# a1q123456/image_stitching

Hardware: AMD Instinct MI355X
Metric: 4K frames stitched/sec (higher is better)
Workload: dtype u8

## Files before the change

image_stitching_amd/csrc/orb.hip:

```cpp
#include "common.h"
#include "dev_math.h"
#include <algorithm>
#include <cmath>
#include <mutex>
#include <unordered_map>

#define ORB_MAX_LEVELS 16
#define ORB_BORDER 32

namespace {

struct LevelDesc {
    int w, h;
    int pp;
    int sp;
    size_t pad_off;
    size_t map_off;
    float scale;
    int nfeat;
    int n2;
    int tiles_x, tiles_y, tile_off;
    int cap1, cand_off;
    int cap2, fin_off;
    int tab_off;
};

struct Levels {
    int n;
    int fast_t, patch, half_patch, edge;
    LevelDesc d[ORB_MAX_LEVELS];
};

struct Work {
    uint8_t *pad, *blur, *score, *nms;
    int* hist;
    int* thr;
    int* tile_cnt;
    uint32_t* surv_xy;
    uint8_t* surv_sc;
    int* cnt1;
    int* cnt2;
    int* flags;
    uint32_t* cand_xy;
    float* cand_resp;
    uint32_t* fin_xy;
    float* fin_resp;
    int* tab;
    int* umax;
    int8_t* pattern;
};

constexpr int ORB_BATCH = 16;
struct OrbIO {
    const uint8_t* src[ORB_BATCH];
    size_t sstride[ORB_BATCH];
    int aligned[ORB_BATCH];
    MisKeyPoint* kps[ORB_BATCH];
    uint32_t* lxy[ORB_BATCH];
    int* n_dev[ORB_BATCH];
    uint8_t* desc[ORB_BATCH];
};
#define WS_OFF(p, f, ws) p = (decltype(p))((const char*)(p) + (size_t)(f) * (ws))

constexpr int GRAY_ROWS = 4;
__global__ __launch_bounds__(256) void gray_kernel(OrbIO io, int w, int h, uint8_t* dst, int pp, size_t ws) {
    const int x = (blockIdx.x * 256 + threadIdx.x) * 4, y0 = blockIdx.y * GRAY_ROWS, f = blockIdx.z;
    if (x >= w) return;
    const uint8_t* bgr = io.src[f];
    const size_t stride = io.sstride[f];
    const int aligned = io.aligned[f];
    WS_OFF(dst, f, ws);
    const int nrows = min(GRAY_ROWS, h - y0);
    if (aligned && x + 4 <= w) {
        unsigned w0[GRAY_ROWS], w1[GRAY_ROWS], w2[GRAY_ROWS];
#pragma unroll
        for (int r = 0; r < GRAY_ROWS; r++) {
            const unsigned* sp = reinterpret_cast<const unsigned*>(bgr + (size_t)min(y0 + r, h - 1) * stride + 3 * (size_t)x);
            w0[r] = sp[0]; w1[r] = sp[1]; w2[r] = sp[2];
        }
#pragma unroll
        for (int r = 0; r < GRAY_ROWS; r++) {
            if (r >= nrows) break;
            const unsigned g0 = ((w0[r] & 255) * 3735 + ((w0[r] >> 8) & 255) * 19235 + ((w0[r] >> 16) & 255) * 9798 + (1 << 14)) >> 15;
            const unsigned g1 = ((w0[r] >> 24) * 3735 + (w1[r] & 255) * 19235 + ((w1[r] >> 8) & 255) * 9798 + (1 << 14)) >> 15;
            const unsigned g2 = (((w1[r] >> 16) & 255) * 3735 + (w1[r] >> 24) * 19235 + (w2[r] & 255) * 9798 + (1 << 14)) >> 15;
            const unsigned g3 = (((w2[r] >> 8) & 255) * 3735 + ((w2[r] >> 16) & 255) * 19235 + (w2[r] >> 24) * 9798 + (1 << 14)) >> 15;
            *reinterpret_cast<unsigned*>(dst + (size_t)(y0 + r + ORB_BORDER) * pp + ORB_BORDER + x) = g0 | (g1 << 8) | (g2 << 16) | (g3 << 24);
        }
    } else {
        for (int r = 0; r < nrows; r++) {
            const uint8_t* s = bgr + (size_t)(y0 + r) * stride + 3 * (size_t)x;
            uint8_t* o = dst + (size_t)(y0 + r + ORB_BORDER) * pp + ORB_BORDER + x;
            for (int k = 0; k < 4 && x + k < w; k++) o[k] = (uint8_t)((s[3 * k] * 3735 + s[3 * k + 1] * 19235 + s[3 * k + 2] * 9798 + (1 << 14)) >> 15);
        }
    }
}

__device__ __forceinline__ unsigned byte_at(unsigned w0, unsigned w1, unsigned w2, int o) {
    const unsigned long long lo = (unsigned long long)w0 | ((unsigned long long)w1 << 32);
    return (o < 8 ? (unsigned)(lo >> (8 * o)) : (w2 >> (8 * (o - 8)))) & 255u;
}
#ifndef MIS_RS_ROWS
#define MIS_RS_ROWS 4
#endif
constexpr int RS_ROWS = MIS_RS_ROWS;
__global__ __launch_bounds__(256) void resize_kernel(const uint8_t* __restrict__ src, int sw, int sh, int spp, uint8_t* __restrict__ dst, int dw, int dh, int dpp,
                                                     const int* __restrict__ tab, size_t ws) {
    const int x = (blockIdx.x * 64 + (threadIdx.x & 63)) * 4;
    const int ybase = __builtin_amdgcn_readfirstlane((blockIdx.y * 4 + (threadIdx.x >> 6)) * RS_ROWS);
    if (x >= dw || ybase >= dh) return;
    WS_OFF(src, blockIdx.z, ws); WS_OFF(dst, blockIdx.z, ws);
    const int dw4 = (dw + 3) & ~3;
    const int *xo = tab, *xm = tab + dw4, *yo = tab + 2 * dw4, *ym = tab + 2 * dw4 + dh;
    const int4 o4 = *reinterpret_cast<const int4*>(xo + x), m4 = *reinterpret_cast<const int4*>(xm + x);
    const int xs[4] = {o4.x, o4.y, o4.z, o4.w}, ms[4] = {m4.x, m4.y, m4.z, m4.w};
    const int nvalid = min(4, dw - x), nrows = min(RS_ROWS, dh - ybase);
    const int base = xs[0] & ~3, last = xs[nvalid - 1] + 1 - base;
    const uint8_t* r0[RS_ROWS];
    const uint8_t* r1[RS_ROWS];
    int my1[RS_ROWS];
#pragma unroll
    for (int r = 0; r < RS_ROWS; r++) {
        const int y = min(ybase + r, dh - 1);
        const int y0 = yo[y], y1 = y0 + 1 < sh ? y0 + 1 : y0;
        my1[r] = ym[y];
        r0[r] = src + (size_t)(y0 + ORB_BORDER) * spp + ORB_BORDER;
        r1[r] = src + (size_t)(y1 + ORB_BORDER) * spp + ORB_BORDER;
    }
    uint8_t* out = dst + (size_t)(ybase + ORB_BORDER) * dpp + ORB_BORDER + x;
    unsigned res[RS_ROWS];
    if (last <= 11) {
        unsigned a[RS_ROWS][3], b[RS_ROWS][3];
#pragma unroll
        for (int r = 0; r < RS_ROWS; r++) {
            const unsigned* p0 = reinterpret_cast<const unsigned*>(r0[r] + base);
            const unsigned* p1 = reinterpret_cast<const unsigned*>(r1[r] + base);
            a[r][0] = p0[0]; a[r][1] = p0[1]; a[r][2] = p0[2]; b[r][0] = p1[0]; b[r][1] = p1[1]; b[r][2] = p1[2];
        }
#pragma unroll
        for (int r = 0; r < RS_ROWS; r++) res[r] = 0;
#pragma unroll
        for (int k = 0; k < 4; k++) {
            const int o = xs[k] - base, mx1 = ms[k], mx0 = 256 - mx1;
            const bool ok = k < nvalid;
            const int oo = ok ? o : 0;
            const bool p1 = oo >= 4, p2 = oo >= 8;
#pragma unroll
            for (int r = 0; r < RS_ROWS; r++) {
                const unsigned alo = p2 ? a[r][2] : (p1 ? a[r][1] : a[r][0]), ahi = p2 ? 0u : (p1 ? a[r][2] : a[r][1]);
                const unsigned blo = p2 ? b[r][2] : (p1 ? b[r][1] : b[r][0]), bhi = p2 ? 0u : (p1 ? b[r][2] : b[r][1]);
                const unsigned ta = __builtin_amdgcn_alignbyte(ahi, alo, (unsigned)oo & 3u), tb = __builtin_amdgcn_alignbyte(bhi, blo, (unsigned)oo & 3u);
                const unsigned h0 = (ta & 255u) * mx0 + ((ta >> 8) & 255u) * mx1;
                const unsigned h1 = (tb & 255u) * mx0 + ((tb >> 8) & 255u) * mx1;
                res[r] |= ok ? ((h0 * (256 - my1[r]) + h1 * my1[r] + (1u << 15)) >> 16) << (8 * k) : 0u;
            }
        }
    } else {
#pragma unroll
        for (int r = 0; r < RS_ROWS; r++) {
            res[r] = 0;
#pragma unroll
            for (int k = 0; k < 4; k++) {
                if (k >= nvalid) break;
                const int x0 = xs[k], x1 = x0 + 1 < sw ? x0 + 1 : x0, mx1 = ms[k], mx0 = 256 - mx1;
                const unsigned h0 = (unsigned)r0[r][x0] * mx0 + (unsigned)r0[r][x1] * mx1;
                const unsigned h1 = (unsigned)r1[r][x0] * mx0 + (unsigned)r1[r][x1] * mx1;
                res[r] |= ((h0 * (256 - my1[r]) + h1 * my1[r] + (1u << 15)) >> 16) << (8 * k);
            }
        }
    }
#pragma unroll
    for (int r = 0; r < RS_ROWS; r++) {
        if (r >= nrows) break;
        uint8_t* o = out + (size_t)r * dpp;
        if (nvalid == 4) *reinterpret_cast<unsigned*>(o) = res[r];
        else
            for (int k = 0; k < nvalid; k++) o[k] = (uint8_t)(res[r] >> (8 * k));
    }
}

template <bool SIDES>
__global__ __launch_bounds__(256) void border_kernel(Levels L, uint8_t* pad, size_t ws) {
    const int f = blockIdx.z / L.n;
    const LevelDesc& d = L.d[blockIdx.z - f * L.n];
    WS_OFF(pad, f, ws);
    const int B = ORB_BORDER, pw = d.w + 2 * B, ph = d.h + 2 * B;
    uint8_t* p = pad + d.pad_off;
    if (!SIDES) {
        const int px4 = (blockIdx.x * 256 + threadIdx.x) * 4;
        if (px4 >= pw) return;
        const bool inner = px4 >= B && px4 + 3 < B + d.w;
        unsigned v[4];
        size_t drow[4], srow[4];
#pragma unroll
        for (int r = 0; r < 4; r++) {
            const int yy = blockIdx.y * 4 + r, py = yy < B ? yy : ph - 2 * B + yy;
            srow[r] = (size_t)(mis_reflect101(py - B, d.h) + B) * d.pp; drow[r] = (size_t)py * d.pp;
        }
        if (inner) {
#pragma unroll
            for (int r = 0; r < 4; r++) v[r] = *reinterpret_cast<const unsigned*>(p + srow[r] + px4);
#pragma unroll
            for (int r = 0; r < 4; r++) *reinterpret_cast<unsigned*>(p + drow[r] + px4) = v[r];
        } else {
#pragma unroll
            for (int r = 0; r < 4; r++)
                for (int k = 0; k < 4 && px4 + k < pw; k++) p[drow[r] + px4 + k] = p[srow[r] + mis_reflect101(px4 + k - B, d.w) + B];
        }
        return;
    }
    const int t = blockIdx.x * 256 + threadIdx.x, row = t >> 4, g = t & 15;
    if (row >= d.h) return;
    const int px = g < 8 ? 4 * g : pw - B + 4 * (g - 8);
    const size_t ro = (size_t)(row + B) * d.pp;
    unsigned v = 0;
#pragma unroll
    for (int k = 0; k < 4; k++) v |= (unsigned)p[ro + mis_reflect101(px + k - B, d.w) + B] << (8 * k);
    if ((px & 3) == 0) *reinterpret_cast<unsigned*>(p + ro + px) = v;
    else
#pragma unroll
        for (int k = 0; k < 4; k++) p[ro + px + k] = (uint8_t)(v >> (8 * k));
}

__device__ __forceinline__ bool fast_pretest(const uint8_t* p, int pp, int t) {
    const int v = p[0], hi = v + t, lo = v - t;
    const int c0 = p[3 * pp], c4 = p[3], c8 = p[-3 * pp], c12 = p[-3];
    unsigned br = (c0 > hi) | ((c4 > hi) << 2) | ((c8 > hi) << 4) | ((c12 > hi) << 6);
    unsigned dk = (c0 < lo) | ((c4 < lo) << 2) | ((c8 < lo) << 4) | ((c12 < lo) << 6);
    const unsigned adj_b = br & ((br >> 2) | (br << 6)), adj_d = dk & ((dk >> 2) | (dk << 6));
    if (!((adj_b | adj_d) & 0x55)) return false;
    const int c2 = p[2 * pp + 2], c6 = p[-2 * pp + 2], c10 = p[-2 * pp - 2], c14 = p[2 * pp - 2];
    br |= ((c2 > hi) << 1) | ((c6 > hi) << 3) | ((c10 > hi) << 5) | ((c14 > hi) << 7);
    dk |= ((c2 < lo) << 1) | ((c6 < lo) << 3) | ((c10 < lo) << 5) | ((c14 < lo) << 7);
    const unsigned b2 = br | (br << 8), d2 = dk | (dk << 8);
    const unsigned rb = b2 & (b2 >> 1) & (b2 >> 2) & (b2 >> 3), rd = d2 & (d2 >> 1) & (d2 >> 2) & (d2 >> 3);
    return ((rb | rd) & 0xff) != 0;
}
__device__ __forceinline__ int fast_score_full(const uint8_t* p, int pp, int t) {
    const int v = p[0];
    int d[16];
    d[0] = v - p[3 * pp]; d[1] = v - p[3 * pp + 1]; d[2] = v - p[2 * pp + 2]; d[3] = v - p[pp + 3];
    d[4] = v - p[3]; d[5] = v - p[-pp + 3]; d[6] = v - p[-2 * pp + 2]; d[7] = v - p[-3 * pp + 1];
    d[8] = v - p[-3 * pp]; d[9] = v - p[-3 * pp - 1]; d[10] = v - p[-2 * pp - 2]; d[11] = v - p[-pp - 3];
    d[12] = v - p[-3]; d[13] = v - p[pp - 3]; d[14] = v - p[2 * pp - 2]; d[15] = v - p[3 * pp - 1];
    int n3[16], x3[16];
#pragma unroll
    for (int i = 0; i < 16; i++) {
        n3[i] = min(min(d[i], d[(i + 1) & 15]), d[(i + 2) & 15]);
        x3[i] = max(max(d[i], d[(i + 1) & 15]), d[(i + 2) & 15]);
    }
    int A = -512, Bm = 512;
#pragma unroll
    for (int i = 0; i < 16; i++) {
        A = max(A, min(min(n3[i], n3[(i + 3) & 15]), n3[(i + 6) & 15]));
        Bm = min(Bm, max(max(x3[i], x3[(i + 3) & 15]), x3[(i + 6) & 15]));
    }
    const int best = max(A, -Bm);
    return best > t ? best - 1 : 0;
}
__device__ __forceinline__ int fast_score_px(const uint8_t* p, int pp, int t) { return fast_pretest(p, pp, t) ? fast_score_full(p, pp, t) : 0; }

#ifndef MIS_FT_ROWS
#define MIS_FT_ROWS 64
#endif
constexpr int FT_COLS = 64, FT_ROWS = MIS_FT_ROWS, FG_PITCH = 96, FG_COL0 = 15, HIST_COPIES = 8;
constexpr int FT_WR = (FT_ROWS + 2 + 3) / 4;
constexpr int FT_SLOTS = FT_COLS * FT_ROWS / 4;
#ifdef MIS_ORB_STATS
__device__ unsigned long long g_orb_stats[8];
#endif
__global__ __launch_bounds__(256) void fast_nms_kernel(Levels L, const uint8_t* pad, int* hist, int* tile_cnt, uint32_t* surv_xy, uint8_t* surv_sc, size_t ws) {
    __shared__ __attribute__((aligned(16))) uint8_t g[(FT_ROWS + 10) * FG_PITCH];
    __shared__ __attribute__((aligned(16))) uint8_t sc[(FT_ROWS + 2) * (FT_COLS + 4)];
    __shared__ int lh[256];
    __shared__ int lcount;
    __shared__ uint32_t lxy[FT_SLOTS];
    __shared__ uint8_t lsc[FT_SLOTS];
    __shared__ unsigned short queue[(FT_ROWS + 2) * (FT_COLS + 2)];
    __shared__ int qcount;
    const int fz = blockIdx.z / L.n, lz = blockIdx.z - fz * L.n;
    const LevelDesc& d = L.d[lz];
    const int x0 = blockIdx.x * FT_COLS, y0 = blockIdx.y * FT_ROWS, t = threadIdx.x;
    if (x0 >= d.w || y0 >= d.h) return;
    WS_OFF(pad, fz, ws); WS_OFF(hist, fz, ws); WS_OFF(tile_cnt, fz, ws); WS_OFF(surv_xy, fz, ws); WS_OFF(surv_sc, fz, ws);
    lh[t] = 0;
    if (t == 0) { lcount = 0; qcount = 0; }
    {
        const int ph = d.h + 2 * ORB_BORDER;
        const uint8_t* src = pad + d.pad_off;
        const int px0 = x0 - 16 + ORB_BORDER, py0 = y0 - 4 + ORB_BORDER;
        for (int i = t; i < (FT_ROWS + 8) * (FG_PITCH / 16); i += 256) {
            const int r = i / (FG_PITCH / 16), c = i - r * (FG_PITCH / 16);
            const int py = min(py0 + r, ph - 1);
            int px = px0 + 16 * c;
            if (px + 15 >= d.pp) px = d.pp - 16;
            reinterpret_cast<uint4*>(g)[i] = *reinterpret_cast<const uint4*>(src + (size_t)py * d.pp + px);
        }
    }
    __syncthreads();
    const int SP = FT_COLS + 4;
    for (int i = t; i < (FT_ROWS + 2) * SP / 4; i += 256) reinterpret_cast<unsigned*>(sc)[i] = 0u;
    {
        const int wv = __builtin_amdgcn_readfirstlane(t >> 6), lane = t & 63;
        const unsigned ft = (unsigned)L.fast_t;
        const int r0 = FT_WR * wv;
        bool pass[FT_WR + 1];
        unsigned long long ball[FT_WR + 1];
        int total = 0;
        {
            const uint8_t* colp = g + r0 * FG_PITCH + (lane + FG_COL0);
            unsigned col[FT_WR + 6];
#pragma unroll
            for (int j = 0; j < FT_WR + 6; j++) col[j] = colp[j * FG_PITCH];
            const int x = x0 - 1 + lane;
            const bool xin = x >= 3 && x < d.w - 3;
            const uint8_t* rowp = g + (r0 + 3) * FG_PITCH + (lane + FG_COL0 - 3);
#pragma unroll
            for (int k = 0; k < FT_WR; k++) {
                const int r = r0 + k, y = y0 - 1 + r;
                const bool rowok = r < FT_ROWS + 2 && y >= 3 && y < d.h - 3;
                const unsigned v = col[k + 3];
                const unsigned dv = max(__builtin_amdgcn_sad_u8(col[k + 6], v, 0u), __builtin_amdgcn_sad_u8(col[k], v, 0u));
                const unsigned dh = max(__builtin_amdgcn_sad_u8(rowp[k * FG_PITCH + 6], v, 0u), __builtin_amdgcn_sad_u8(rowp[k * FG_PITCH], v, 0u));
                pass[k] = rowok & xin & (min(dv, dh) > ft);
                ball[k] = __ballot(pass[k]);
                total += __popcll(ball[k]);
            }
        }
        {
            const int k = lane >> 1, cc = FT_COLS + (lane & 1), r = r0 + k, y = y0 - 1 + r, x = x0 - 1 + cc;
            bool ps = false;
            if (lane < 2 * FT_WR && r < FT_ROWS + 2) {
                const uint8_t* pp = g + (r + 3) * FG_PITCH + (cc + FG_COL0);
                const unsigned v = pp[0];
                const unsigned dv = max(__builtin_amdgcn_sad_u8(pp[3 * FG_PITCH], v, 0u), __builtin_amdgcn_sad_u8(pp[-3 * FG_PITCH], v, 0u));
                const unsigned dh = max(__builtin_amdgcn_sad_u8(pp[3], v, 0u), __builtin_amdgcn_sad_u8(pp[-3], v, 0u));
                ps = x >= 3 && x < d.w - 3 && y >= 3 && y < d.h - 3 && min(dv, dh) > ft;
            }
            pass[FT_WR] = ps;
            ball[FT_WR] = __ballot(ps);
            total += __popcll(ball[FT_WR]);
        }
        int base = 0;
        if (lane == 0 && total) base = atomicAdd(&qcount, total);
        base = __builtin_amdgcn_readfirstlane(base);
        const unsigned long long below = (1ull << lane) - 1ull;
#pragma unroll
        for (int k = 0; k < FT_WR + 1; k++) {
            if (pass[k]) {
                const int r = k < FT_WR ? r0 + k : r0 + (lane >> 1), c = k < FT_WR ? lane : FT_COLS + (lane & 1);
                queue[base + __popcll(ball[k] & below)] = (unsigned short)(r * (FT_COLS + 2) + c);
            }
            base += __popcll(ball[k]);
        }
    }
    __syncthreads();
    for (int q = t; q < qcount; q += 256) {
        const int i = queue[q], r = i / (FT_COLS + 2), c = i - r * (FT_COLS + 2);
        const int fsv = fast_score_full(g + (r + 3) * FG_PITCH + (c + FG_COL0), FG_PITCH, L.fast_t);
        sc[r * SP + c] = (uint8_t)fsv;
#ifdef MIS_ORB_STATS
        if (fsv) atomicAdd(&g_orb_stats[3], 1ull);
#endif
    }
    __syncthreads();
    {
        const int nq = qcount;
        for (int q0 = 0; q0 < nq; q0 += 256) {
            const int q = q0 + t;
            bool keep = false;
            int x = 0, y = 0, v = 0;
            if (q < nq) {
                const int i = queue[q], r = i / (FT_COLS + 2), c = i - r * (FT_COLS + 2);
                const uint8_t* s_ = sc + r * SP + c;
                v = s_[0];
                x = x0 - 1 + c; y = y0 - 1 + r;
                keep = v && r >= 1 && r <= FT_ROWS && c >= 1 && c <= FT_COLS && x >= L.edge && x < d.w - L.edge && y >= L.edge && y < d.h - L.edge &&
                       v > s_[-1] && v > s_[1] && v > s_[-SP - 1] && v > s_[-SP] && v > s_[-SP + 1] && v > s_[SP - 1] && v > s_[SP] && v > s_[SP + 1];
            }
            const unsigned long long m = __ballot(keep);
            int base = 0;
            if ((t & 63) == 0 && m) base = atomicAdd(&lcount, __popcll(m));
            base = __shfl(base, 0);
            if (keep) {
                const int j = base + __popcll(m & ((1ull << (t & 63)) - 1ull));
                lxy[j] = (uint32_t)x | ((uint32_t)y << 16); lsc[j] = (uint8_t)v;
            }
        }
    }
    __syncthreads();
    const int n = lcount;
    const int tile = d.tile_off + blockIdx.y * d.tiles_x + blockIdx.x;
    if (t == 0) tile_cnt[tile] = n;
    if (n == 0) return;
    for (int j = t; j < n; j += 256) {
        atomicAdd(&lh[lsc[j]], 1);
        surv_xy[(size_t)tile * FT_SLOTS + j] = lxy[j]; surv_sc[(size_t)tile * FT_SLOTS + j] = lsc[j];
    }
    __syncthreads();
    if (lh[t]) atomicAdd(&hist[((lz * HIST_COPIES) + ((blockIdx.x + blockIdx.y) & (HIST_COPIES - 1))) * 256 + t], lh[t]);
}

__global__ __launch_bounds__(256) void fast_cut_kernel(Levels L, const int* hist, int* thr, int* flags, size_t ws) {
    __shared__ int suf[256];
    __shared__ int s_thr;
    const int l = blockIdx.x, t = threadIdx.x;
    WS_OFF(hist, blockIdx.y, ws); WS_OFF(thr, blockIdx.y, ws); WS_OFF(flags, blockIdx.y, ws);
    const LevelDesc& d = L.d[l];
    int hsum = 0;
    for (int c = 0; c < HIST_COPIES; c++) hsum += hist[(l * HIST_COPIES + c) * 256 + t];
    suf[t] = t ? hsum : 0;
    __syncthreads();
    for (int o = 1; o < 256; o <<= 1) {
        int add = t + o < 256 ? suf[t + o] : 0;
        __syncthreads();
        suf[t] += add;
        __syncthreads();
    }
    if (t == 0) s_thr = d.n2 == 0 ? 256 : 1;
    __syncthreads();
    if (d.n2 > 0 && suf[1] > d.n2 && t >= 1 && suf[t] >= d.n2 && (t == 255 || suf[t + 1] < d.n2)) s_thr = t;
    __syncthreads();
    if (t == 0) {
        thr[l] = s_thr;
        if (s_thr < 256 && suf[s_thr] > d.cap1) atomicOr(&flags[0], 1);
    }
}

constexpr int CT_TILES = 16;
__global__ __launch_bounds__(256) void compact_kernel(Levels L, const int* tile_cnt, const uint32_t* surv_xy, const uint8_t* surv_sc, const int* thr,
                                                      int* cnt1, uint32_t* cand_xy, float* cand_resp, size_t ws) {
    __shared__ int s_cnt[CT_TILES], s_off[CT_TILES];
    __shared__ int s_base;
    const int l = blockIdx.y, t = threadIdx.x, lane = t & 63, wave = t >> 6;
    WS_OFF(tile_cnt, blockIdx.z, ws); WS_OFF(surv_xy, blockIdx.z, ws); WS_OFF(surv_sc, blockIdx.z, ws); WS_OFF(thr, blockIdx.z, ws);
    WS_OFF(cnt1, blockIdx.z, ws); WS_OFF(cand_xy, blockIdx.z, ws); WS_OFF(cand_resp, blockIdx.z, ws);
    const LevelDesc& d = L.d[l];
    const int ntiles = d.tiles_x * d.tiles_y, first = blockIdx.x * CT_TILES;
    if (first >= ntiles) return;
    const int th = thr[l];
    for (int k = 0; k < CT_TILES / 4; k++) {
        const int slot = wave * (CT_TILES / 4) + k, til = first + slot;
        int cnt = 0;
        if (til < ntiles) {
            const int tile = d.tile_off + til, n = tile_cnt[tile];
            for (int j0 = 0; j0 < n; j0 += 64) {
                const int j = j0 + lane;
                const int v = j < n ? surv_sc[(size_t)tile * FT_SLOTS + j] : 0;
                cnt += __popcll(__ballot(v >= th && v > 0));
            }
        }
        if (lane == 0) s_cnt[slot] = cnt;
    }
    __syncthreads();
    if (t == 0) {
        int tot = 0;
        for (int k = 0; k < CT_TILES; k++) { s_off[k] = tot; tot += s_cnt[k]; }
        s_base = tot ? atomicAdd(&cnt1[l], tot) : 0;
    }
    __syncthreads();
    for (int k = 0; k < CT_TILES / 4; k++) {
        const int slot = wave * (CT_TILES / 4) + k, til = first + slot;
        if (til >= ntiles || s_cnt[slot] == 0) continue;
        const int tile = d.tile_off + til, n = tile_cnt[tile];
        int run = s_base + s_off[slot];
        for (int j0 = 0; j0 < n; j0 += 64) {
            const int j = j0 + lane;
            const int v = j < n ? surv_sc[(size_t)tile * FT_SLOTS + j] : 0;
            const bool keep = v >= th && v > 0;
            const unsigned long long m = __ballot(keep);
            if (keep) {
                const int i = run + __popcll(m & ((1ull << lane) - 1ull));
                if (i < d.cap1) { cand_xy[d.cand_off + i] = surv_xy[(size_t)tile * FT_SLOTS + j]; cand_resp[d.cand_off + i] = (float)v; }
            }
            run += __popcll(m);
        }
    }
}

__global__ void nms_raster_kernel(LevelDesc d, const int* tile_cnt, const uint32_t* surv_xy, const uint8_t* surv_sc, uint8_t* nms) {
    const int ntiles = d.tiles_x * d.tiles_y;
    for (int tl = blockIdx.x; tl < ntiles; tl += gridDim.x) {
        const int tile = d.tile_off + tl, n = tile_cnt[tile];
        for (int j = threadIdx.x; j < n; j += blockDim.x) {
            uint32_t xy = surv_xy[(size_t)tile * FT_SLOTS + j];
            nms[d.map_off + (size_t)(xy >> 16) * d.sp + (xy & 0xffff)] = surv_sc[(size_t)tile * FT_SLOTS + j];
        }
    }
}

__global__ __launch_bounds__(256) void harris_kernel(Levels L, const uint8_t* pad, const int* cnt1, const uint32_t* cand_xy, float* cand_resp, size_t ws) {
    const LevelDesc& d = L.d[blockIdx.y];
    WS_OFF(pad, blockIdx.z, ws); WS_OFF(cnt1, blockIdx.z, ws); WS_OFF(cand_xy, blockIdx.z, ws); WS_OFF(cand_resp, blockIdx.z, ws);
    int i = blockIdx.x * 256 + threadIdx.x;
    int n = min(cnt1[blockIdx.y], d.cap1);
    if (i >= n) return;
    uint32_t xy = cand_xy[d.cand_off + i];
    int x = xy & 0xffff, y = xy >> 16;
    const int pp = d.pp;
    const uint8_t* q0 = pad + d.pad_off + (size_t)(y + ORB_BORDER - 4) * pp + (x + ORB_BORDER - 4);
    const unsigned sh = (unsigned)((uintptr_t)q0 & 3u);
    const uint8_t* a0 = q0 - sh;
    int px[9][9];
#pragma unroll
    for (int r = 0; r < 9; r++) {
        const unsigned* row = reinterpret_cast<const unsigned*>(a0 + (size_t)r * pp);
        const unsigned d0 = row[0], d1 = row[1], d2 = row[2];
        const unsigned w0 = __builtin_amdgcn_alignbyte(d1, d0, sh), w1 = __builtin_amdgcn_alignbyte(d2, d1, sh), w2 = __builtin_amdgcn_alignbyte(0u, d2, sh);
#pragma unroll
        for (int k = 0; k < 4; k++) { px[r][k] = (int)((w0 >> (8 * k)) & 255u); px[r][4 + k] = (int)((w1 >> (8 * k)) & 255u); }
        px[r][8] = (int)(w2 & 255u);
    }
    int a = 0, b = 0, c = 0;
#pragma unroll
    for (int by = 0; by < 7; by++)
#pragma unroll
        for (int bx = 0; bx < 7; bx++) {
            const int Ix = (px[by + 1][bx + 2] - px[by + 1][bx]) * 2 + (px[by][bx + 2] - px[by][bx]) + (px[by + 2][bx + 2] - px[by + 2][bx]);
            const int Iy = (px[by + 2][bx + 1] - px[by][bx + 1]) * 2 + (px[by + 2][bx] - px[by][bx]) + (px[by + 2][bx + 2] - px[by][bx + 2]);
            a += Ix * Ix; b += Iy * Iy; c += Ix * Iy;
        }
    const float scale = 1.f / ((1 << 2) * 7 * 255.f);
// ... 423 lines not shown
        d.w = (int)lrint((double)((float)w / sc));
        d.h = (int)lrint((double)((float)h / sc));
        d.pp = (int)mis_align_up((size_t)d.w + 2 * ORB_BORDER, 64);
        d.sp = (int)mis_align_up((size_t)d.w, 64);
        d.pad_off = pad_off; pad_off += (size_t)d.pp * (d.h + 2 * ORB_BORDER);
        d.map_off = map_off; map_off += (size_t)d.sp * d.h;
        if (l < L.n - 1) { d.nfeat = (int)lrintf(nd); sum += d.nfeat; nd *= factor; }
        else d.nfeat = std::max(p.nfeatures - sum, 0);
        d.n2 = p.score_type == 0 ? 2 * d.nfeat : d.nfeat;
        d.tiles_x = (d.w + FT_COLS - 1) / FT_COLS; d.tiles_y = (d.h + FT_ROWS - 1) / FT_ROWS;
        d.tile_off = surv_off; surv_off += d.tiles_x * d.tiles_y;
        d.cap1 = 4 * d.n2 + 4096;
        d.cap2 = std::min(d.nfeat + 128, 2048);
        d.cand_off = cand_off; cand_off += d.cap1;
        d.fin_off = fin_off; fin_off += d.cap2;
        d.tab_off = tab_off; tab_off += (2 * ((d.w + 3) & ~3) + 2 * d.h + 3) & ~3;
    }
    o->pad_bytes = pad_off; o->map_bytes = map_off; o->cand_total = cand_off; o->fin_total = fin_off; o->tab_total = tab_off; o->surv_total = surv_off;
    o->tab_host.assign(tab_off, 0);
    for (int l = 1; l < L.n; l++) {
        int* t = o->tab_host.data() + L.d[l].tab_off;
        const int dw4 = (L.d[l].w + 3) & ~3;
        linear_exact_coeffs(L.d[l].w, L.d[l - 1].w, t, t + dw4);
        linear_exact_coeffs(L.d[l].h, L.d[l - 1].h, t + 2 * dw4, t + 2 * dw4 + L.d[l].h);
    }
}

int upload_tables(MisOrb* o) {
    MisContext* ctx = o->ctx;
    if (o->tab_total)
        MIS_HIP(ctx, hipMemcpyAsync(o->w.tab, o->tab_host.data(), sizeof(int) * o->tab_total, hipMemcpyHostToDevice, ctx->stream));
    MIS_HIP(ctx, hipStreamSynchronize(ctx->stream));
    return MIS_OK;
}

std::mutex g_feat_mutex;
std::unordered_map<void*, size_t> g_feat_sizes;

int alloc_features(MisContext* ctx, int cap, int desc_cols, int desc_dtype, MisFeatures* f) {
    size_t kb = mis_align_up(sizeof(MisKeyPoint) * (size_t)cap, 256), db = mis_align_up((size_t)cap * desc_cols * mis_dtype_size(desc_dtype), 256);
    size_t lb = mis_align_up(sizeof(uint32_t) * (size_t)cap, 256);
    void* mem = nullptr;
    size_t got = 0;
    int rc = mis_pool_alloc(ctx, kb + db + lb + 256, &mem, &got);
    if (rc != MIS_OK) return rc;
    f->keypoints = (MisKeyPoint*)mem;
    f->descriptors = (uint8_t*)mem + kb;
    f->desc_cols = desc_cols; f->desc_dtype = desc_dtype;
    f->owner_ = mem;
    f->n = 0;
    std::lock_guard<std::mutex> lock(g_feat_mutex);
    g_feat_sizes[mem] = got;
    return MIS_OK;
}

inline uint32_t* feat_lxy(const MisFeatures* f, int cap) {
    size_t kb = mis_align_up(sizeof(MisKeyPoint) * (size_t)cap, 256), db = mis_align_up((size_t)cap * f->desc_cols * mis_dtype_size(f->desc_dtype), 256);
    return (uint32_t*)((uint8_t*)f->owner_ + kb + db);
}
inline int* feat_count(const MisFeatures* f, int cap) {
    size_t kb = mis_align_up(sizeof(MisKeyPoint) * (size_t)cap, 256), db = mis_align_up((size_t)cap * f->desc_cols * mis_dtype_size(f->desc_dtype), 256);
    size_t lb = mis_align_up(sizeof(uint32_t) * (size_t)cap, 256);
    return (int*)((uint8_t*)f->owner_ + kb + db + lb);
}

int enqueue_detect_group(MisOrb* o, const DevImage* img, int w, int h, MisFeatures* out, int ng) {
    MisContext* ctx = o->ctx;
    const Levels& L = o->L;
    const Work& W = o->w;
    hipStream_t st = ctx->stream;
    const LevelDesc& d0 = L.d[0];
    const size_t ws = o->ws_stride;
    const unsigned nf = (unsigned)ng;
    OrbIO io;
    for (int k = 0; k < ORB_BATCH; k++) {
        const int q = k < ng ? k : 0;
        io.src[k] = (const uint8_t*)img[q].data; io.sstride[k] = img[q].stride;
        io.aligned[k] = (img[q].stride % 4 == 0) && ((uintptr_t)img[q].data % 4 == 0);
        io.kps[k] = out[q].keypoints; io.lxy[k] = feat_lxy(&out[q], o->out_cap); io.n_dev[k] = feat_count(&out[q], o->out_cap);
        io.desc[k] = (uint8_t*)out[q].descriptors;
    }
    MIS_HIP(ctx, hipMemset2DAsync(W.hist, ws ? ws : sizeof(int) * (256 * HIST_COPIES * ORB_MAX_LEVELS + 4 * ORB_MAX_LEVELS), 0,
                                  sizeof(int) * (256 * HIST_COPIES * ORB_MAX_LEVELS + 4 * ORB_MAX_LEVELS), nf, st));
    hipLaunchKernelGGL(gray_kernel, dim3((w + 1023) / 1024, (h + GRAY_ROWS - 1) / GRAY_ROWS, nf), dim3(256), 0, st, io, w, h, W.pad + d0.pad_off, d0.pp, ws);
    for (int l = 1; l < L.n; l++) {
        const LevelDesc &s = L.d[l - 1], &d = L.d[l];
        hipLaunchKernelGGL(resize_kernel, dim3((d.w + 255) / 256, (d.h + 4 * RS_ROWS - 1) / (4 * RS_ROWS), nf), dim3(256), 0, st, W.pad + s.pad_off, s.w, s.h, s.pp, W.pad + d.pad_off, d.w,
                           d.h, d.pp, W.tab + d.tab_off, ws);
    }
    const int pw0 = d0.w + 2 * ORB_BORDER, ph0 = d0.h + 2 * ORB_BORDER;
    hipLaunchKernelGGL((border_kernel<true>), dim3((d0.h * 16 + 255) / 256, 1, L.n * nf), dim3(256), 0, st, L, W.pad, ws);
    hipLaunchKernelGGL((border_kernel<false>), dim3((pw0 + 1023) / 1024, 2 * ORB_BORDER / 4, L.n * nf), dim3(256), 0, st, L, W.pad, ws);
    dim3 gmap((d0.w + FT_COLS - 1) / FT_COLS, (d0.h + FT_ROWS - 1) / FT_ROWS, L.n * nf);
    hipLaunchKernelGGL(fast_nms_kernel, gmap, dim3(256), 0, st, L, W.pad, W.hist, W.tile_cnt, W.surv_xy, W.surv_sc, ws);
    hipLaunchKernelGGL(fast_cut_kernel, dim3(L.n, nf), dim3(256), 0, st, L, W.hist, W.thr, W.flags, ws);
    hipLaunchKernelGGL(compact_kernel, dim3((d0.tiles_x * d0.tiles_y + CT_TILES - 1) / CT_TILES, L.n, nf), dim3(256), 0, st, L, W.tile_cnt, W.surv_xy, W.surv_sc, W.thr, W.cnt1,
                       W.cand_xy, W.cand_resp, ws);
    const int use_harris = o->p.score_type == 0;
    if (use_harris)
        hipLaunchKernelGGL(harris_kernel, dim3((L.d[0].cap1 + 255) / 256, L.n, nf), dim3(256), 0, st, L, W.pad, W.cnt1, W.cand_xy, W.cand_resp, ws);
    hipLaunchKernelGGL(select_rank_kernel, dim3(L.n, nf), dim3(1024), 0, st, L, W.cnt1, W.cand_xy, W.cand_resp, W.cnt2, W.fin_xy, W.fin_resp, W.flags,
                       use_harris, ws);
    hipLaunchKernelGGL(assemble_angle_kernel, dim3((o->out_cap + 3) / 4, nf), dim3(256), 0, st, L, W.pad, W.cnt2, W.fin_xy, W.fin_resp, W.umax, io, o->out_cap, ws, o->direct_describe ? 0 : 1);
    if (o->direct_describe) {
        UMax16 um16;
        for (int v = 0; v < 16; v++) um16.v[v] = o->umax_host[v];
        hipLaunchKernelGGL(describe_direct_kernel, dim3((o->out_cap + 3) / 4, nf), dim3(256), 0, st, L, W.pad, io, W.pattern, W.umax, um16, ws);
    } else {
        for (int k = 0; k < ng; k++) {
            hipLaunchKernelGGL(blur_kernel, dim3((pw0 + 63) / 64, (ph0 + 31) / 32, L.n), dim3(256), 0, st, L, W.pad + k * ws, W.blur + k * ws);
            hipLaunchKernelGGL(describe_kernel, dim3((o->out_cap + 7) / 8), dim3(256), 0, st, L, W.blur + k * ws, out[k].keypoints, io.lxy[k], io.n_dev[k], W.pattern,
                               (uint8_t*)out[k].descriptors);
        }
    }
    MIS_HIP(ctx, hipGetLastError());
    return MIS_OK;
}

int check_image(MisOrb* o, const MisImage* bgr) {
    MisContext* ctx = o->ctx;
    MIS_CHECK(ctx, bgr && bgr->data, MIS_E_INVALID, "null image");
    MIS_CHECK(ctx, bgr->dtype == MIS_U8 && bgr->channels == 3, MIS_E_UNSUPPORTED, "ORB input must be 8UC3 (BGR)");
    MIS_CHECK(ctx, bgr->width <= o->max_w && bgr->height <= o->max_h && bgr->width >= 64 && bgr->height >= 64, MIS_E_INVALID,
              "image %dx%d outside the finder's range (64x64 .. %dx%d)", bgr->width, bgr->height, o->max_w, o->max_h);
    return MIS_OK;
}

int replan_if_needed(MisOrb* o, int w, int h) {
    if (w == o->cur_w && h == o->cur_h) return MIS_OK;
    MIS_HIP(o->ctx, hipStreamSynchronize(o->ctx->stream));
    plan_levels(o, w, h);
    o->cur_w = w; o->cur_h = h;
    return upload_tables(o);
}

int orb_alloc_workspace(MisOrb* o, int frames) {
    MisContext* ctx = o->ctx;
    size_t off = 0;
    auto carve = [&](size_t bytes) { size_t o_ = off; off += mis_align_up(bytes, 256); return o_; };
    const bool frame_blur = !o->direct_describe;
    size_t o_pad = carve(o->pad_bytes), o_blur = frame_blur ? carve(o->pad_bytes) : 0;
    size_t o_hist = carve(sizeof(int) * (256 * HIST_COPIES * ORB_MAX_LEVELS + 4 * ORB_MAX_LEVELS)), o_flags = carve(256);
    size_t o_sxy = carve(sizeof(uint32_t) * FT_SLOTS * (size_t)o->surv_total), o_ssc = carve(FT_SLOTS * (size_t)o->surv_total), o_tc = carve(sizeof(int) * (size_t)o->surv_total);
    size_t o_cxy = carve(sizeof(uint32_t) * o->cand_total), o_cr = carve(sizeof(float) * o->cand_total);
    size_t o_fxy = carve(sizeof(uint32_t) * o->fin_total), o_fr = carve(sizeof(float) * o->fin_total);
    size_t o_tab = carve(sizeof(int) * (o->tab_total + 4)), o_umax = carve(sizeof(int) * 64), o_pat = carve(1024);
    const size_t tail = mis_align_up(o->map_bytes, 256) + (frame_blur ? 0 : mis_align_up(o->pad_bytes, 256));
    void* mem = nullptr;
    if (hipMalloc(&mem, off * (size_t)frames + tail) != hipSuccess) return mis_set_error(ctx, MIS_E_NOMEM, "hipMalloc of %zu bytes failed", off * (size_t)frames + tail);
    o->mem = mem; o->ws_stride = off; o->ws_frames = frames;
    uint8_t* m = (uint8_t*)o->mem;
    uint8_t* shared = m + off * (size_t)frames;
    Work& W = o->w;
    W.pad = m + o_pad; W.nms = shared; W.blur = frame_blur ? m + o_blur : shared + mis_align_up(o->map_bytes, 256); W.score = nullptr;
    W.hist = (int*)(m + o_hist); W.thr = W.hist + 256 * HIST_COPIES * ORB_MAX_LEVELS; W.cnt1 = W.thr + ORB_MAX_LEVELS; W.cnt2 = W.cnt1 + ORB_MAX_LEVELS;
    W.surv_xy = (uint32_t*)(m + o_sxy); W.surv_sc = m + o_ssc; W.tile_cnt = (int*)(m + o_tc);
    W.flags = (int*)(m + o_flags);
    W.cand_xy = (uint32_t*)(m + o_cxy); W.cand_resp = (float*)(m + o_cr); W.fin_xy = (uint32_t*)(m + o_fxy); W.fin_resp = (float*)(m + o_fr);
    W.tab = (int*)(m + o_tab); W.umax = (int*)(m + o_umax); W.pattern = (int8_t*)(m + o_pat);
    return MIS_OK;
}

int orb_init_workspace(MisOrb* o) {
    MisContext* ctx = o->ctx;
    const Work& W = o->w;
    MIS_HIP(ctx, hipMemcpyAsync(W.umax, o->umax_host, sizeof(o->umax_host), hipMemcpyHostToDevice, ctx->stream));
    MIS_HIP(ctx, hipMemcpyAsync(W.pattern, o->pattern_host, sizeof(o->pattern_host), hipMemcpyHostToDevice, ctx->stream));
    MIS_HIP(ctx, hipMemset2DAsync(W.flags, o->ws_stride, 0, 256, (size_t)o->ws_frames, ctx->stream));
    MIS_HIP(ctx, hipStreamSynchronize(ctx->stream));
    return upload_tables(o);
}

int orb_ensure_frames(MisOrb* o, int frames) {
    frames = std::min(frames, ORB_BATCH);
    if (o->ws_frames >= frames) return MIS_OK;
    MisContext* ctx = o->ctx;
    MIS_HIP(ctx, hipStreamSynchronize(ctx->stream));
    void* old = o->mem;
    const Work oldw = o->w;
    const size_t olds = o->ws_stride;
    const int oldf = o->ws_frames;
    int rc = MIS_E_NOMEM;
    for (int f = frames; f > oldf; f = std::max(oldf, f / 2)) {
        if ((rc = orb_alloc_workspace(o, f)) == MIS_OK) break;
    }
    if (rc != MIS_OK) {
        o->mem = old; o->w = oldw; o->ws_stride = olds; o->ws_frames = oldf;
        return oldf >= 1 ? MIS_OK : rc;
    }
    if (old) MIS_HIP(ctx, hipFree(old));
    return orb_init_workspace(o);
// ... 241 lines not shown
```

Before: 2716.

## Fuse grayscale conversion and border fill into level-0 FAST tile kernel

```diff
diff --git a/image_stitching_amd/csrc/orb.hip b/image_stitching_amd/csrc/orb.hip
--- a/image_stitching_amd/csrc/orb.hip
+++ b/image_stitching_amd/csrc/orb.hip
@@ -62,59 +62,23 @@
 };
 #define WS_OFF(p, f, ws) p = (decltype(p))((const char*)(p) + (size_t)(f) * (ws))
 
-constexpr int GRAY_ROWS = 4;
-__global__ __launch_bounds__(256) void gray_kernel(OrbIO io, int w, int h, uint8_t* dst, int pp, size_t ws) {
-    const int x = (blockIdx.x * 256 + threadIdx.x) * 4, y0 = blockIdx.y * GRAY_ROWS, f = blockIdx.z;
-    if (x >= w) return;
-    const uint8_t* bgr = io.src[f];
-    const size_t stride = io.sstride[f];
-    const int aligned = io.aligned[f];
-    WS_OFF(dst, f, ws);
-    const int nrows = min(GRAY_ROWS, h - y0);
-    if (aligned && x + 4 <= w) {
-        unsigned w0[GRAY_ROWS], w1[GRAY_ROWS], w2[GRAY_ROWS];
-#pragma unroll
-        for (int r = 0; r < GRAY_ROWS; r++) {
-            const unsigned* sp = reinterpret_cast<const unsigned*>(bgr + (size_t)min(y0 + r, h - 1) * stride + 3 * (size_t)x);
-            w0[r] = sp[0]; w1[r] = sp[1]; w2[r] = sp[2];
-        }
-#pragma unroll
-        for (int r = 0; r < GRAY_ROWS; r++) {
-            if (r >= nrows) break;
-            const unsigned g0 = ((w0[r] & 255) * 3735 + ((w0[r] >> 8) & 255) * 19235 + ((w0[r] >> 16) & 255) * 9798 + (1 << 14)) >> 15;
-            const unsigned g1 = ((w0[r] >> 24) * 3735 + (w1[r] & 255) * 19235 + ((w1[r] >> 8) & 255) * 9798 + (1 << 14)) >> 15;
-            const unsigned g2 = (((w1[r] >> 16) & 255) * 3735 + (w1[r] >> 24) * 19235 + (w2[r] & 255) * 9798 + (1 << 14)) >> 15;
-            const unsigned g3 = (((w2[r] >> 8) & 255) * 3735 + ((w2[r] >> 16) & 255) * 19235 + (w2[r] >> 24) * 9798 + (1 << 14)) >> 15;
-            *reinterpret_cast<unsigned*>(dst + (size_t)(y0 + r + ORB_BORDER) * pp + ORB_BORDER + x) = g0 | (g1 << 8) | (g2 << 16) | (g3 << 24);
-        }
-    } else {
-        for (int r = 0; r < nrows; r++) {
-            const uint8_t* s = bgr + (size_t)(y0 + r) * stride + 3 * (size_t)x;
-            uint8_t* o = dst + (size_t)(y0 + r + ORB_BORDER) * pp + ORB_BORDER + x;
-            for (int k = 0; k < 4 && x + k < w; k++) o[k] = (uint8_t)((s[3 * k] * 3735 + s[3 * k + 1] * 19235 + s[3 * k + 2] * 9798 + (1 << 14)) >> 15);
-        }
-    }
-}
-
-__device__ __forceinline__ unsigned byte_at(unsigned w0, unsigned w1, unsigned w2, int o) {
-    const unsigned long long lo = (unsigned long long)w0 | ((unsigned long long)w1 << 32);
-    return (o < 8 ? (unsigned)(lo >> (8 * o)) : (w2 >> (8 * (o - 8)))) & 255u;
-}
-#ifndef MIS_RS_ROWS
-#define MIS_RS_ROWS 4
-#endif
-constexpr int RS_ROWS = MIS_RS_ROWS;
-__global__ __launch_bounds__(256) void resize_kernel(const uint8_t* __restrict__ src, int sw, int sh, int spp, uint8_t* __restrict__ dst, int dw, int dh, int dpp,
-                                                     const int* __restrict__ tab, size_t ws) {
-    const int x = (blockIdx.x * 64 + (threadIdx.x & 63)) * 4;
-    const int ybase = __builtin_amdgcn_readfirstlane((blockIdx.y * 4 + (threadIdx.x >> 6)) * RS_ROWS);
-    if (x >= dw || ybase >= dh) return;
-    WS_OFF(src, blockIdx.z, ws); WS_OFF(dst, blockIdx.z, ws);
+__device__ __forceinline__ unsigned gray_px(unsigned b, unsigned g, unsigned r) { return (b * 3735 + g * 19235 + r * 9798 + (1 << 14)) >> 15; }
+__device__ __forceinline__ unsigned gray4(unsigned w0, unsigned w1, unsigned w2) {
+    const unsigned g0 = gray_px(w0 & 255, (w0 >> 8) & 255, (w0 >> 16) & 255);
+    const unsigned g1 = gray_px(w0 >> 24, w1 & 255, (w1 >> 8) & 255);
+    const unsigned g2 = gray_px((w1 >> 16) & 255, w1 >> 24, w2 & 255);
+    const unsigned g3 = gray_px((w2 >> 8) & 255, (w2 >> 16) & 255, w2 >> 24);
+    return g0 | (g1 << 8) | (g2 << 16) | (g3 << 24);
+}
+
+constexpr int RS_ROWS = 4;
+__device__ __forceinline__ void resize4(const uint8_t* __restrict__ src, int sw, int sh, int spp, int dw, int dh, const int* __restrict__ tab,
+                                        int x, int ybase, unsigned (&res)[RS_ROWS]) {
     const int dw4 = (dw + 3) & ~3;
     const int *xo = tab, *xm = tab + dw4, *yo = tab + 2 * dw4, *ym = tab + 2 * dw4 + dh;
     const int4 o4 = *reinterpret_cast<const int4*>(xo + x), m4 = *reinterpret_cast<const int4*>(xm + x);
     const int xs[4] = {o4.x, o4.y, o4.z, o4.w}, ms[4] = {m4.x, m4.y, m4.z, m4.w};
-    const int nvalid = min(4, dw - x), nrows = min(RS_ROWS, dh - ybase);
+    const int nvalid = min(4, dw - x);
     const int base = xs[0] & ~3, last = xs[nvalid - 1] + 1 - base;
     const uint8_t* r0[RS_ROWS];
     const uint8_t* r1[RS_ROWS];
@@ -127,8 +91,6 @@
         r0[r] = src + (size_t)(y0 + ORB_BORDER) * spp + ORB_BORDER;
         r1[r] = src + (size_t)(y1 + ORB_BORDER) * spp + ORB_BORDER;
     }
-    uint8_t* out = dst + (size_t)(ybase + ORB_BORDER) * dpp + ORB_BORDER + x;
-    unsigned res[RS_ROWS];
     if (last <= 11) {
         unsigned a[RS_ROWS][3], b[RS_ROWS][3];
 #pragma unroll
@@ -169,6 +131,18 @@
             }
         }
     }
+}
+
+__global__ __launch_bounds__(256) void resize_kernel(const uint8_t* __restrict__ src, int sw, int sh, int spp, uint8_t* __restrict__ dst, int dw, int dh, int dpp,
+                                                     const int* __restrict__ tab, size_t ws) {
+    const int x = (blockIdx.x * 64 + (threadIdx.x & 63)) * 4;
+    const int ybase = __builtin_amdgcn_readfirstlane((blockIdx.y * 4 + (threadIdx.x >> 6)) * RS_ROWS);
+    if (x >= dw || ybase >= dh) return;
+    WS_OFF(src, blockIdx.z, ws); WS_OFF(dst, blockIdx.z, ws);
+    unsigned res[RS_ROWS];
+    resize4(src, sw, sh, spp, dw, dh, tab, x, ybase, res);
+    const int nvalid = min(4, dw - x), nrows = min(RS_ROWS, dh - ybase);
+    uint8_t* out = dst + (size_t)(ybase + ORB_BORDER) * dpp + ORB_BORDER + x;
 #pragma unroll
     for (int r = 0; r < RS_ROWS; r++) {
         if (r >= nrows) break;
@@ -177,49 +151,6 @@
         else
             for (int k = 0; k < nvalid; k++) o[k] = (uint8_t)(res[r] >> (8 * k));
     }
-}
-
-template <bool SIDES>
-__global__ __launch_bounds__(256) void border_kernel(Levels L, uint8_t* pad, size_t ws) {
-    const int f = blockIdx.z / L.n;
-    const LevelDesc& d = L.d[blockIdx.z - f * L.n];
-    WS_OFF(pad, f, ws);
-    const int B = ORB_BORDER, pw = d.w + 2 * B, ph = d.h + 2 * B;
-    uint8_t* p = pad + d.pad_off;
-    if (!SIDES) {
-        const int px4 = (blockIdx.x * 256 + threadIdx.x) * 4;
-        if (px4 >= pw) return;
-        const bool inner = px4 >= B && px4 + 3 < B + d.w;
-        unsigned v[4];
-        size_t drow[4], srow[4];
-#pragma unroll
-        for (int r = 0; r < 4; r++) {
-            const int yy = blockIdx.y * 4 + r, py = yy < B ? yy : ph - 2 * B + yy;
-            srow[r] = (size_t)(mis_reflect101(py - B, d.h) + B) * d.pp; drow[r] = (size_t)py * d.pp;
-        }
-        if (inner) {
-#pragma unroll
-            for (int r = 0; r < 4; r++) v[r] = *reinterpret_cast<const unsigned*>(p + srow[r] + px4);
-#pragma unroll
-            for (int r = 0; r < 4; r++) *reinterpret_cast<unsigned*>(p + drow[r] + px4) = v[r];
-        } else {
-#pragma unroll
-            for (int r = 0; r < 4; r++)
-                for (int k = 0; k < 4 && px4 + k < pw; k++) p[drow[r] + px4 + k] = p[srow[r] + mis_reflect101(px4 + k - B, d.w) + B];
-        }
-        return;
-    }
-    const int t = blockIdx.x * 256 + threadIdx.x, row = t >> 4, g = t & 15;
-    if (row >= d.h) return;
-    const int px = g < 8 ? 4 * g : pw - B + 4 * (g - 8);
-    const size_t ro = (size_t)(row + B) * d.pp;
-    unsigned v = 0;
-#pragma unroll
-    for (int k = 0; k < 4; k++) v |= (unsigned)p[ro + mis_reflect101(px + k - B, d.w) + B] << (8 * k);
-    if ((px & 3) == 0) *reinterpret_cast<unsigned*>(p + ro + px) = v;
-    else
-#pragma unroll
-        for (int k = 0; k < 4; k++) p[ro + px + k] = (uint8_t)(v >> (8 * k));
 }
 
 __device__ __forceinline__ bool fast_pretest(const uint8_t* p, int pp, int t) {
@@ -266,10 +197,13 @@
 constexpr int FT_COLS = 64, FT_ROWS = MIS_FT_ROWS, FG_PITCH = 96, FG_COL0 = 15, HIST_COPIES = 8;
 constexpr int FT_WR = (FT_ROWS + 2 + 3) / 4;
 constexpr int FT_SLOTS = FT_COLS * FT_ROWS / 4;
+constexpr int FW_GROUPS = (FT_COLS + 8) / 4, FW_QUADS = (FT_ROWS + 8) / 4;
+static_assert(FT_ROWS % 4 == 0, "the level-0 window is built from 4 x 4 pixel items");
 #ifdef MIS_ORB_STATS
 __device__ unsigned long long g_orb_stats[8];
 #endif
-__global__ __launch_bounds__(256) void fast_nms_kernel(Levels L, const uint8_t* pad, int* hist, int* tile_cnt, uint32_t* surv_xy, uint8_t* surv_sc, size_t ws) {
+template <bool LEVEL0>
+__global__ __launch_bounds__(256) void level_fast_kernel(Levels L, OrbIO io, uint8_t* pad, int* hist, int* tile_cnt, uint32_t* surv_xy, uint8_t* surv_sc, size_t ws) {
     __shared__ __attribute__((aligned(16))) uint8_t g[(FT_ROWS + 10) * FG_PITCH];
     __shared__ __attribute__((aligned(16))) uint8_t sc[(FT_ROWS + 2) * (FT_COLS + 4)];
     __shared__ int lh[256];
@@ -278,14 +212,63 @@
     __shared__ uint8_t lsc[FT_SLOTS];
     __shared__ unsigned short queue[(FT_ROWS + 2) * (FT_COLS + 2)];
     __shared__ int qcount;
-    const int fz = blockIdx.z / L.n, lz = blockIdx.z - fz * L.n;
-    const LevelDesc& d = L.d[lz];
-    const int x0 = blockIdx.x * FT_COLS, y0 = blockIdx.y * FT_ROWS, t = threadIdx.x;
-    if (x0 >= d.w || y0 >= d.h) return;
+    const int fz = blockIdx.y;
+    int lv = 0, tix = blockIdx.x;
+    if (!LEVEL0) {
+        tix += L.d[1].tile_off;
+        for (lv = 1; lv < L.n - 1 && tix >= L.d[lv + 1].tile_off; lv++) {}
+        tix -= L.d[lv].tile_off;
+    }
+    const LevelDesc& d = L.d[lv];
+    const int tyi = tix / d.tiles_x, txi = tix - tyi * d.tiles_x;
+    const int x0 = txi * FT_COLS, y0 = tyi * FT_ROWS, t = threadIdx.x;
+    const int x1 = min(x0 + FT_COLS, d.w), y1 = min(y0 + FT_ROWS, d.h);
     WS_OFF(pad, fz, ws); WS_OFF(hist, fz, ws); WS_OFF(tile_cnt, fz, ws); WS_OFF(surv_xy, fz, ws); WS_OFF(surv_sc, fz, ws);
+    uint8_t* lev = pad + d.pad_off + (size_t)ORB_BORDER * d.pp + ORB_BORDER;
     lh[t] = 0;
     if (t == 0) { lcount = 0; qcount = 0; }
-    {
+    if (LEVEL0) {
+        const uint8_t* bgr = io.src[fz];
+        const size_t stride = io.sstride[fz];
+        const int aligned = io.aligned[fz];
+        for (int i = t; i < FW_GROUPS * FW_QUADS; i += 256) {
+            const int q = i / FW_GROUPS, cg = i - q * FW_GROUPS;
+            const int x = x0 - 4 + 4 * cg, yb = y0 - 4 + 4 * q;
+            if (x < 0 || x >= d.w || yb < 0 || yb >= d.h) continue;
+            const int nvalid = min(4, d.w - x), nrows = min(4, d.h - yb);
+            unsigned res[4];
+            if (aligned && nvalid == 4) {
+                unsigned w0[4], w1[4], w2[4];
+#pragma unroll
+                for (int r = 0; r < 4; r++) {
+                    const unsigned* sp = reinterpret_cast<const unsigned*>(bgr + (size_t)min(yb + r, d.h - 1) * stride + 3 * (size_t)x);
+                    w0[r] = sp[0]; w1[r] = sp[1]; w2[r] = sp[2];
+                }
+#pragma unroll
+                for (int r = 0; r < 4; r++) res[r] = gray4(w0[r], w1[r], w2[r]);
+            } else {
+                for (int r = 0; r < 4; r++) {
+                    res[r] = 0;
+                    if (r >= nrows) continue;
+                    const uint8_t* sp = bgr + (size_t)(yb + r) * stride + 3 * (size_t)x;
+                    for (int k = 0; k < nvalid; k++) res[r] |= gray_px(sp[3 * k], sp[3 * k + 1], sp[3 * k + 2]) << (8 * k);
+                }
+            }
+            const bool own_x = x >= x0 && x < x1;
+#pragma unroll
+            for (int r = 0; r < 4; r++) {
+                if (r >= nrows) break;
+                const int y = yb + r;
+                *reinterpret_cast<unsigned*>(g + (y - y0 + 4) * FG_PITCH + (x - x0 + 16)) = res[r];
+                if (own_x && y >= y0 && y < y1) {
+                    uint8_t* o = lev + (size_t)y * d.pp + x;
+                    if (nvalid == 4) *reinterpret_cast<unsigned*>(o) = res[r];
+                    else
+                        for (int k = 0; k < nvalid; k++) o[k] = (uint8_t)(res[r] >> (8 * k));
+                }
+            }
+        }
+    } else {
         const int ph = d.h + 2 * ORB_BORDER;
         const uint8_t* src = pad + d.pad_off;
         const int px0 = x0 - 16 + ORB_BORDER, py0 = y0 - 4 + ORB_BORDER;
@@ -298,6 +281,33 @@
         }
     }
     __syncthreads();
+    {
+        auto win = [&](int x, int y) { return g[(y - y0 + 4) * FG_PITCH + (x - x0 + 16)]; };
+        const bool xedge = x0 <= ORB_BORDER || x1 >= d.w - ORB_BORDER - 1, yedge = y0 <= ORB_BORDER || y1 >= d.h - ORB_BORDER - 1;
+        if (xedge)
+            for (int i = t; i < FT_ROWS * 2 * ORB_BORDER; i += 256) {
+                const int y = y0 + i / (2 * ORB_BORDER), j = i % (2 * ORB_BORDER);
+                const int px = j < ORB_BORDER ? j - ORB_BORDER : d.w + j - ORB_BORDER;
+                const int sx = mis_reflect101(px, d.w);
+                if (y < y1 && sx >= x0 && sx < x1) lev[(size_t)y * d.pp + px] = win(sx, y);
+            }
+        if (yedge)
+            for (int i = t; i < 2 * ORB_BORDER * (FT_COLS + 2 * ORB_BORDER); i += 256) {
+                const int j = i / (FT_COLS + 2 * ORB_BORDER), k = i % (FT_COLS + 2 * ORB_BORDER);
+                const int py = j < ORB_BORDER ? j - ORB_BORDER : d.h + j - ORB_BORDER;
+                const int sy = mis_reflect101(py, d.h);
+                if (sy < y0 || sy >= y1) continue;
+                int px, sx;
+                if (k < FT_COLS) { px = sx = x0 + k; if (px >= x1) continue; }
+                else {
+                    if (!xedge) continue;
+                    px = k < FT_COLS + ORB_BORDER ? k - FT_COLS - ORB_BORDER : d.w + k - FT_COLS - ORB_BORDER;
+                    sx = mis_reflect101(px, d.w);
+                    if (sx < x0 || sx >= x1) continue;
+                }
+                lev[(size_t)py * d.pp + px] = win(sx, sy);
+            }
+    }
     const int SP = FT_COLS + 4;
     for (int i = t; i < (FT_ROWS + 2) * SP / 4; i += 256) reinterpret_cast<unsigned*>(sc)[i] = 0u;
     {
@@ -390,7 +400,7 @@
     }
     __syncthreads();
     const int n = lcount;
-    const int tile = d.tile_off + blockIdx.y * d.tiles_x + blockIdx.x;
+    const int tile = d.tile_off + tix;
     if (t == 0) tile_cnt[tile] = n;
     if (n == 0) return;
     for (int j = t; j < n; j += 256) {
@@ -398,7 +408,7 @@
         surv_xy[(size_t)tile * FT_SLOTS + j] = lxy[j]; surv_sc[(size_t)tile * FT_SLOTS + j] = lsc[j];
     }
     __syncthreads();
-    if (lh[t]) atomicAdd(&hist[((lz * HIST_COPIES) + ((blockIdx.x + blockIdx.y) & (HIST_COPIES - 1))) * 256 + t], lh[t]);
+    if (lh[t]) atomicAdd(&hist[((lv * HIST_COPIES) + ((txi + tyi) & (HIST_COPIES - 1))) * 256 + t], lh[t]);
 }
 
 __global__ __launch_bounds__(256) void fast_cut_kernel(Levels L, const int* hist, int* thr, int* flags, size_t ws) {
@@ -428,16 +438,26 @@
 }
 
 constexpr int CT_TILES = 16;
+inline int compact_blocks(const Levels& L) {
+    int nb = 0;
+    for (int l = 0; l < L.n; l++) nb += (L.d[l].tiles_x * L.d[l].tiles_y + CT_TILES - 1) / CT_TILES;
+    return nb;
+}
 __global__ __launch_bounds__(256) void compact_kernel(Levels L, const int* tile_cnt, const uint32_t* surv_xy, const uint8_t* surv_sc, const int* thr,
                                                       int* cnt1, uint32_t* cand_xy, float* cand_resp, size_t ws) {
     __shared__ int s_cnt[CT_TILES], s_off[CT_TILES];
     __shared__ int s_base;
-    const int l = blockIdx.y, t = threadIdx.x, lane = t & 63, wave = t >> 6;
-    WS_OFF(tile_cnt, blockIdx.z, ws); WS_OFF(surv_xy, blockIdx.z, ws); WS_OFF(surv_sc, blockIdx.z, ws); WS_OFF(thr, blockIdx.z, ws);
-    WS_OFF(cnt1, blockIdx.z, ws); WS_OFF(cand_xy, blockIdx.z, ws); WS_OFF(cand_resp, blockIdx.z, ws);
+    const int t = threadIdx.x, lane = t & 63, wave = t >> 6;
+    WS_OFF(tile_cnt, blockIdx.y, ws); WS_OFF(surv_xy, blockIdx.y, ws); WS_OFF(surv_sc, blockIdx.y, ws); WS_OFF(thr, blockIdx.y, ws);
+    WS_OFF(cnt1, blockIdx.y, ws); WS_OFF(cand_xy, blockIdx.y, ws); WS_OFF(cand_resp, blockIdx.y, ws);
+    int l = 0, blk = blockIdx.x;
+    for (; l < L.n - 1; l++) {
+        const int nb = (L.d[l].tiles_x * L.d[l].tiles_y + CT_TILES - 1) / CT_TILES;
+        if (blk < nb) break;
+        blk -= nb;
+    }
     const LevelDesc& d = L.d[l];
-    const int ntiles = d.tiles_x * d.tiles_y, first = blockIdx.x * CT_TILES;
-    if (first >= ntiles) return;
+    const int ntiles = d.tiles_x * d.tiles_y, first = blk * CT_TILES;
     const int th = thr[l];
     for (int k = 0; k < CT_TILES / 4; k++) {
         const int slot = wave * (CT_TILES / 4) + k, til = first + slot;
@@ -1027,19 +1047,16 @@
     }
     MIS_HIP(ctx, hipMemset2DAsync(W.hist, ws ? ws : sizeof(int) * (256 * HIST_COPIES * ORB_MAX_LEVELS + 4 * ORB_MAX_LEVELS), 0,
                                   sizeof(int) * (256 * HIST_COPIES * ORB_MAX_LEVELS + 4 * ORB_MAX_LEVELS), nf, st));
-    hipLaunchKernelGGL(gray_kernel, dim3((w + 1023) / 1024, (h + GRAY_ROWS - 1) / GRAY_ROWS, nf), dim3(256), 0, st, io, w, h, W.pad + d0.pad_off, d0.pp, ws);
+    hipLaunchKernelGGL(level_fast_kernel<true>, dim3(d0.tiles_x * d0.tiles_y, nf), dim3(256), 0, st, L, io, W.pad, W.hist, W.tile_cnt, W.surv_xy, W.surv_sc, ws);
     for (int l = 1; l < L.n; l++) {
         const LevelDesc &s = L.d[l - 1], &d = L.d[l];
         hipLaunchKernelGGL(resize_kernel, dim3((d.w + 255) / 256, (d.h + 4 * RS_ROWS - 1) / (4 * RS_ROWS), nf), dim3(256), 0, st, W.pad + s.pad_off, s.w, s.h, s.pp, W.pad + d.pad_off, d.w,
                            d.h, d.pp, W.tab + d.tab_off, ws);
     }
-    const int pw0 = d0.w + 2 * ORB_BORDER, ph0 = d0.h + 2 * ORB_BORDER;
-    hipLaunchKernelGGL((border_kernel<true>), dim3((d0.h * 16 + 255) / 256, 1, L.n * nf), dim3(256), 0, st, L, W.pad, ws);
-    hipLaunchKernelGGL((border_kernel<false>), dim3((pw0 + 1023) / 1024, 2 * ORB_BORDER / 4, L.n * nf), dim3(256), 0, st, L, W.pad, ws);
-    dim3 gmap((d0.w + FT_COLS - 1) / FT_COLS, (d0.h + FT_ROWS - 1) / FT_ROWS, L.n * nf);
-    hipLaunchKernelGGL(fast_nms_kernel, gmap, dim3(256), 0, st, L, W.pad, W.hist, W.tile_cnt, W.surv_xy, W.surv_sc, ws);
+    if (L.n > 1)
+        hipLaunchKernelGGL(level_fast_kernel<false>, dim3(o->surv_total - L.d[1].tile_off, nf), dim3(256), 0, st, L, io, W.pad, W.hist, W.tile_cnt, W.surv_xy, W.surv_sc, ws);
     hipLaunchKernelGGL(fast_cut_kernel, dim3(L.n, nf), dim3(256), 0, st, L, W.hist, W.thr, W.flags, ws);
-    hipLaunchKernelGGL(compact_kernel, dim3((d0.tiles_x * d0.tiles_y + CT_TILES - 1) / CT_TILES, L.n, nf), dim3(256), 0, st, L, W.tile_cnt, W.surv_xy, W.surv_sc, W.thr, W.cnt1,
+    hipLaunchKernelGGL(compact_kernel, dim3(compact_blocks(L), nf), dim3(256), 0, st, L, W.tile_cnt, W.surv_xy, W.surv_sc, W.thr, W.cnt1,
                        W.cand_xy, W.cand_resp, ws);
     const int use_harris = o->p.score_type == 0;
     if (use_harris)
@@ -1052,6 +1069,7 @@
         for (int v = 0; v < 16; v++) um16.v[v] = o->umax_host[v];
         hipLaunchKernelGGL(describe_direct_kernel, dim3((o->out_cap + 3) / 4, nf), dim3(256), 0, st, L, W.pad, io, W.pattern, W.umax, um16, ws);
     } else {
+        const int pw0 = d0.w + 2 * ORB_BORDER, ph0 = d0.h + 2 * ORB_BORDER;
         for (int k = 0; k < ng; k++) {
             hipLaunchKernelGGL(blur_kernel, dim3((pw0 + 63) / 64, (ph0 + 31) / 32, L.n), dim3(256), 0, st, L, W.pad + k * ws, W.blur + k * ws);
             hipLaunchKernelGGL(describe_kernel, dim3((o->out_cap + 7) / 8), dim3(256), 0, st, L, W.blur + k * ws, out[k].keypoints, io.lxy[k], io.n_dev[k], W.pattern,
```

Result: no change. 2707 (median of 6 runs) (-0.3%).
